# dobrosketchkun/dither_pie

Measured on AMD Instinct MI355X. Metric: Mpixel/s dither+quantize @4K 256-color (Bayer 8x8 + nearest-palette, uint8 RGB in/out), higher is better.
Workload: dtype u8; 1 GPU; C2: Bayer 8x8 + 256-colour nearest palette palr(256,7), 3840x2160 RGB, 24 distinct frames rnd(2160,3840,1234+i) per GPU resident in HBM, frames sharded per rank; frames_per_gpu=24, h=2160, w=3840, colors=256, matrix=8x8, parallelism=frames x1

## Files before the change

dither_pie_amd/csrc/host_sanitize.cpp:

```cpp
#include <cstdio>
#include <cstdlib>
#include <cstring>
#include <string>

#include "host_logic.h"
#include "ordered_plan.h"
#include "ordered_fine.h"

using namespace dp;

static std::vector<double> read_pts(const char *path, int K)
{
    std::vector<double> p((size_t)K * 3);
    FILE *f = fopen(path, "rb");
    if (!f || fread(p.data(), sizeof(double), p.size(), f) != p.size()) {
        fprintf(stderr, "cannot read %d points from %s\n", K, path);
        exit(2);
    }
    fclose(f);
    return p;
}

static uint32_t lcg(uint32_t &s)
{
// ... 623 lines not shown
    const int mw = 8;
    std::vector<uint32_t> coord4(K), tm, nm;
    for (int j = 0; j < K; ++j) coord4[j] = (uint32_t)pal[3 * j] | ((uint32_t)pal[3 * j + 1] << 8) | ((uint32_t)pal[3 * j + 2] << 16);
    fine_masks(pal, K, mw, tm, nm);
    FineTable ft, again;
    fine_pack(tm.data(), nm.data(), mw, K, coord4, fine_table_fits, ft);
    fine_pack(tm.data(), nm.data(), mw, K, coord4, fine_table_fits, again);
    const std::vector<uint32_t> im = ft.ok ? ft.lds_image() : std::vector<uint32_t>();
    int bad = ft.ok != again.ok || ft.off != again.off || ft.win_idx != again.win_idx || ft.wide_idx != again.wide_idx;
    if (ft.ok) bad += (int64_t)im.size() * 4 != fine_table_bytes(ft.n_win, ft.n_wide) || !fine_table_fits(ft.n_win, ft.n_wide);
    f = fopen(out_path, "wb");
    if (!f) return 2;
    const int32_t head[4] = {ft.ok ? 1 : 0, ft.n_win, ft.n_wide, (int32_t)im.size()};
    fwrite(head, sizeof(int32_t), 4, f);
    if (ft.ok) {
        fwrite(ft.off.data(), 2, ft.off.size(), f);
        fwrite(ft.win_idx.data(), 2, ft.win_idx.size(), f);
        fwrite(ft.wide_cell.data(), 2, ft.wide_cell.size(), f);
        fwrite(ft.wide_idx.data(), 2, ft.wide_idx.size(), f);
        fwrite(ft.quad.data(), 4, ft.quad.size(), f);
        fwrite(ft.pair.data(), 4, ft.pair.size(), f);
        fwrite(ft.wide.data(), 4, ft.wide.size(), f);
        fwrite(im.data(), 4, im.size(), f);
    }
    fclose(f);
    printf("finepack K=%d ok=%d windows=%d wide=%d bytes=%lld bad=%d\n", K, (int)ft.ok, ft.n_win, ft.n_wide,
           (long long)(ft.ok ? fine_table_bytes(ft.n_win, ft.n_wide) : 0), bad);
    return bad ? 1 : 0;
}

static int run_fineplan(const char *path, const int n_cases)
{
    FILE *f = fopen(path, "rb");
    if (!f) {
        fprintf(stderr, "cannot open %s\n", path);
        return 2;
    }
    for (int c = 0; c < n_cases; ++c) {
        OrderedFacts facts;
        OrderedSwitches sw;
        FineFacts ff;
        if (fread(&facts, sizeof(facts), 1, f) != 1 || fread(&sw, sizeof(sw), 1, f) != 1 || fread(&ff, sizeof(ff), 1, f) != 1 || facts.hw < 1 ||
            facts.w < 1 || facts.n_cus < 1) {
            fprintf(stderr, "bad record %d in %s\n", c, path);
            return 2;
        }
        const OrderedPlan p = plan_ordered(facts, sw);
        printf("fine %d %s %d\n", c, family_name(p.family), (int)fine_replaces(p, ff));
    }
    fclose(f);
    return 0;
}

static int run_voidcluster(const char *path, const int n_cases)
{
    FILE *f = fopen(path, "rb");
    if (!f) {
        fprintf(stderr, "cannot open %s\n", path);
        return 2;
    }
    for (int c = 0; c < n_cases; ++c) {
        int32_t head[4];
        if (fread(head, sizeof(int32_t), 4, f) != 4 || !vac_args_ok(head[0], head[1], head[3])) {
            fprintf(stderr, "bad record %d in %s\n", c, path);
            return 2;
        }
        const int n = head[0] * head[1];
        std::vector<uint16_t> ranks((size_t)n);
        std::vector<float> thr((size_t)n);
        int rounds = 0;
        vac_generate(head[0], head[1], (uint32_t)head[2], head[3], ranks.data(), &rounds);
        vac_thresholds(ranks.data(), n, thr.data());
        printf("ranks %d %d", c, rounds);
        for (int i = 0; i < n; ++i) printf(" %u", (unsigned)ranks[(size_t)i]);
        printf("\nthr %d", c);
        for (int i = 0; i < n; ++i) {
            uint32_t bits;
            std::memcpy(&bits, &thr[(size_t)i], sizeof(bits));
            printf(" %08x", bits);
        }
        printf("\n");
    }
    fclose(f);
    return 0;
}

static int run_metric(const char *path, const int n_cases)
{
    FILE *f = fopen(path, "rb");
    if (!f) {
        fprintf(stderr, "cannot open %s\n", path);
        return 2;
    }
    for (int c = 0; c < n_cases; ++c) {
        int32_t head[2];
        if (fread(head, sizeof(int32_t), 2, f) != 2 || head[0] < 1 || head[0] > 256 || head[1] < 0 || head[1] > (1 << 20)) {
            fprintf(stderr, "bad record %d in %s\n", c, path);
            return 2;
        }
        const int K = head[0], n = head[1];
        std::vector<float> pal((size_t)3 * K), thr((size_t)n);
        std::vector<uint8_t> rgb((size_t)3 * n);
        if (fread(pal.data(), sizeof(float), pal.size(), f) != pal.size() || fread(thr.data(), sizeof(float), thr.size(), f) != thr.size() ||
            fread(rgb.data(), 1, rgb.size(), f) != rgb.size() || !metric_palette_ok(pal.data(), K)) {
            fprintf(stderr, "bad record %d in %s\n", c, path);
            return 2;
// ... 32 lines not shown
            fprintf(stderr, "bad record %d in %s\n", c, path);
            return 2;
        }
        IdiffPlan p;
        const int rc = idiff_plan(dx.data(), dy.data(), wt.data(), head[0], head[1], head[2], p);
        printf("idiff %d %d %d %d", c, rc, p.n, p.skew);
        for (int k = 0; k < p.n; ++k) printf(" %u", (unsigned)p.q[k]);
        printf("\n");
    }
    fclose(f);
    return 0;
}

static int run_okfit(const char *path, const int n_cases)
{
    FILE *f = fopen(path, "rb");
    if (!f) {
        fprintf(stderr, "cannot open %s\n", path);
        return 2;
    }
    for (int c = 0; c < n_cases; ++c) {
        int32_t head[3];
        if (fread(head, sizeof(int32_t), 3, f) != 3 || head[0] < 0 || head[0] > (1 << 24)) {
            fprintf(stderr, "bad record %d in %s\n", c, path);
            return 2;
        }
        const size_t n = (size_t)head[0];
        std::vector<uint32_t> codes(n), counts(n);
        if (fread(codes.data(), sizeof(uint32_t), n, f) != n || fread(counts.data(), sizeof(uint32_t), n, f) != n) {
            fprintf(stderr, "bad record %d in %s\n", c, path);
            return 2;
        }
        const int K = head[1], rule = okfit_check(codes.data(), counts.data(), (int64_t)n, K, head[2]);
        printf("okfit %d %d", c, rule);
        if (!rule) {
            std::vector<uint8_t> pal((size_t)3 * K);
            std::vector<int32_t> centres((size_t)3 * K);
            int n_iter = 0;
            uint64_t distortion = 0;
            okfit_host(codes.data(), counts.data(), (int64_t)n, K, head[2], pal.data(), centres.data(), &n_iter, &distortion);
            printf(" %d %llu", n_iter, (unsigned long long)distortion);
            for (int i = 0; i < 3 * K; ++i) printf(" %u", (unsigned)pal[(size_t)i]);
            for (int i = 0; i < 3 * K; ++i) printf(" %d", centres[(size_t)i]);
        }
        printf("\n");
    }
    fclose(f);
    return 0;
}

int main(int argc, char **argv)
{
    if (argc < 4) {
        fprintf(stderr, "usage: %s kdtree|edtables|accel <pts.f64> <K> [bw]  |  mediancut <rgb.u8> <n> <depth>  |  indexmap <lists.bin> <n>  |  giflzw <cases.bin> <n>  |  pngdeflate|pngdyn|pngfile <cases.bin> <n>  |  orderedplan <cases.bin> <n>  |  voidcluster <cases.bin> <n>  |  metric <cases.bin> <n>  |  finepack <pal.u8> <K> <out.bin>  |  fineplan <cases.bin> <n>  |  idiffplan <cases.bin> <n>  |  okfit <cases.bin> <n>\n", argv[0]);
        return 2;
    }
    if (std::string(argv[1]) == "mediancut") return run_mediancut(argv[2], atol(argv[3]), argc > 4 ? atoi(argv[4]) : 4);
    if (std::string(argv[1]) == "indexmap") return run_indexmap(argv[2], atoi(argv[3]));
    if (std::string(argv[1]) == "giflzw") return run_giflzw(argv[2], atoi(argv[3]));
    if (std::string(argv[1]) == "pngdeflate") return run_pngdeflate(argv[2], atoi(argv[3]), false);
    if (std::string(argv[1]) == "pngdyn") return run_pngdeflate(argv[2], atoi(argv[3]), true);
    if (std::string(argv[1]) == "pngfile") return run_pngfile(argv[2], atoi(argv[3]));
    if (std::string(argv[1]) == "orderedplan") return run_orderedplan(argv[2], atoi(argv[3]));
    if (std::string(argv[1]) == "voidcluster") return run_voidcluster(argv[2], atoi(argv[3]));
    if (std::string(argv[1]) == "metric") return run_metric(argv[2], atoi(argv[3]));
    if (std::string(argv[1]) == "finepack") return argc > 4 ? run_finepack(argv[2], atoi(argv[3]), argv[4]) : 2;
    if (std::string(argv[1]) == "fineplan") return run_fineplan(argv[2], atoi(argv[3]));
    if (std::string(argv[1]) == "idiffplan") return run_idiffplan(argv[2], atoi(argv[3]));
    if (std::string(argv[1]) == "okfit") return run_okfit(argv[2], atoi(argv[3]));
    const int K = atoi(argv[3]);
    if (K < 1 || K > 1024) return 2;
    const std::vector<double> pts = read_pts(argv[2], K);
    const std::string cmd = argv[1];
    if (cmd == "kdtree") return run_kdtree(pts, K);
    if (cmd == "edtables") return run_edtables(pts, K);
    if (cmd == "accel") return run_accel(pts, K, argc > 4 ? atoi(argv[4]) : 8);
    return 2;
}
```

dither_pie_amd/csrc/ordered.hip:

```cpp
#include <type_traits>

#include "dp_internal.h"
#include "ordered_plan.h"
#include "ordered_fine.h"
#include "tree_query.hip.h"

namespace dp {

namespace {

constexpr int kListCap = 16384;
constexpr int kLdsTreeK = 256;
constexpr int kLdsTreeNodes = 512;
constexpr int kDrainAt = kListCap - kBlock * 64;

struct Geo {
    uint32_t n_px;
    uint32_t hw, w, h;
    double inv_hw, inv_w;
    int y0, x0;
    int ty0, tx0;
    int aligned;
    int neg2;
    uint32_t adv_y, adv_x;
// ... 1763 lines not shown
        drain_b(qb < 64u ? qb : 64u);
    }
}


__device__ __forceinline__ void cand6(const uint32_t x, const uint4 ca, const uint32_t c4, const uint32_t c5, const int neg2, int &m0,
                                      int &m1, int &m2)
{
    int n0, n1, n2, n3, n4, n5, p0, p1, p2, p3, p4, p5;
    asm volatile(
        "v_dot4_u32_u8 %[n0], %[c0], %[c0], 0\n\t"
        "v_dot4_u32_u8 %[p0], %[x], %[c0], 0\n\t"
        "v_dot4_u32_u8 %[n1], %[c1], %[c1], 0\n\t"
        "v_dot4_u32_u8 %[p1], %[x], %[c1], 0\n\t"
        "v_dot4_u32_u8 %[n2], %[c2], %[c2], 0\n\t"
        "v_dot4_u32_u8 %[p2], %[x], %[c2], 0\n\t"
        "v_dot4_u32_u8 %[n3], %[c3], %[c3], 0\n\t"
        "v_dot4_u32_u8 %[p3], %[x], %[c3], 0\n\t"
        "v_dot4_u32_u8 %[n4], %[c4], %[c4], 0\n\t"
        "v_dot4_u32_u8 %[p4], %[x], %[c4], 0\n\t"
        "v_dot4_u32_u8 %[n5], %[c5], %[c5], 0\n\t"
        "v_dot4_u32_u8 %[p5], %[x], %[c5], 0\n\t"
        "v_lshl_add_u32 %[n0], %[n0], 8, 0\n\t"
        "v_lshl_add_u32 %[n1], %[n1], 8, 4\n\t"
        "v_lshl_add_u32 %[n2], %[n2], 8, 8\n\t"
        "v_lshl_add_u32 %[n3], %[n3], 8, 12\n\t"
        "v_lshl_add_u32 %[n4], %[n4], 8, 16\n\t"
        "v_lshl_add_u32 %[n5], %[n5], 8, 20\n\t"
        "v_mad_i32_i24 %[n0], %[p0], %[ng], %[n0]\n\t"
        "v_mad_i32_i24 %[n1], %[p1], %[ng], %[n1]\n\t"
        "v_mad_i32_i24 %[n2], %[p2], %[ng], %[n2]\n\t"
        "v_mad_i32_i24 %[n3], %[p3], %[ng], %[n3]\n\t"
        "v_mad_i32_i24 %[n4], %[p4], %[ng], %[n4]\n\t"
        "v_mad_i32_i24 %[n5], %[p5], %[ng], %[n5]\n\t"
        "v_min3_i32 %[m0], %[n0], %[n1], %[n2]\n\t"
        "v_med3_i32 %[m1], %[n0], %[n1], %[n2]\n\t"
        "v_max3_i32 %[m2], %[n0], %[n1], %[n2]\n\t"
        "v_med3_i32 %[m2], %[m1], %[m2], %[n3]\n\t"
        "v_med3_i32 %[m1], %[m0], %[m1], %[n3]\n\t"
        "v_min_i32 %[m0], %[m0], %[n3]\n\t"
        "v_med3_i32 %[m2], %[m1], %[m2], %[n4]\n\t"
        "v_med3_i32 %[m1], %[m0], %[m1], %[n4]\n\t"
        "v_min_i32 %[m0], %[m0], %[n4]\n\t"
        "v_med3_i32 %[m2], %[m1], %[m2], %[n5]\n\t"
        "v_med3_i32 %[m1], %[m0], %[m1], %[n5]\n\t"
        "v_min_i32 %[m0], %[m0], %[n5]\n\t"
        : [n0] "=&v"(n0), [n1] "=&v"(n1), [n2] "=&v"(n2), [n3] "=&v"(n3), [n4] "=&v"(n4), [n5] "=&v"(n5), [p0] "=&v"(p0),
          [p1] "=&v"(p1), [p2] "=&v"(p2), [p3] "=&v"(p3), [p4] "=&v"(p4), [p5] "=&v"(p5), [m0] "=&v"(m0), [m1] "=&v"(m1),
          [m2] "=&v"(m2)
        : [x] "v"(x), [c0] "v"(ca.x), [c1] "v"(ca.y), [c2] "v"(ca.z), [c3] "v"(ca.w), [c4] "v"(c4), [c5] "v"(c5),
          [ng] "s"(neg2));
}

__device__ __forceinline__ uint32_t fine_cell_offset(const uint32_t x)
{
    return ((x >> 2) & 0x3eu) | ((x >> 5) & 0x7c0u) | ((x >> 8) & 0xf800u);
}

struct FineLds {
    uint32_t wide_at, pair_at, off_at, ids_at, thr_at;
};

template <int MODE>
__device__ __forceinline__ uint32_t fine_pixel_full(const uint32_t entry, const uint8_t *__restrict__ in, uint8_t *__restrict__ out,
                                                    unsigned long long *__restrict__ flags, const Geo &g, const PalDev &pal,
                                                    const ThrDev &thr, const uint32_t *s_words, const FineLds &at)
{
    const uint32_t mask = entry & 15u;
    const uint32_t p = (entry >> 4) * 4u + (uint32_t)__builtin_ctz(mask | 16u);
    const uint8_t *s_bytes = reinterpret_cast<const uint8_t *>(s_words);
    const uint8_t *b = in + (size_t)p * 3;
    const uint32_t x = (uint32_t)b[0] | ((uint32_t)b[1] << 8) | ((uint32_t)b[2] << 16);
    LeanThr th;
    pixel_threshold<MODE>(p, g, thr, s_words + at.thr_at / 4, 0.0f, 0.0f, 0.0f, th);
    const uint32_t cell2 = fine_cell_offset(x);
    uint32_t c = 0;
    bool done = false, slow = false;
    if (*reinterpret_cast<const uint16_t *>(s_bytes + at.off_at + cell2) == 0) {
        const uint16_t *ids = reinterpret_cast<const uint16_t *>(s_bytes + at.ids_at);
        const uint32_t cell = cell2 >> 1;
        uint32_t lo = 0;
#pragma unroll
        for (uint32_t step = kFineIds / 2; step != 0u; step >>= 1)
            if ((uint32_t)ids[lo + step] <= cell) lo += step;
        done = resolve_wide<MODE>(x, th, thr.sh, s_words + at.wide_at / 4 + lo * kWideList, kWideList, c);
    }
    if (!done) {
        bool hard;
        Leaf lf;
        leaf_find_global<8>(x, pal, lf);
        c = resolve_pixel<MODE, 8>(x, th, lf, g, pal, thr, nullptr, slow, hard);
    }
    uint8_t *o = out + (size_t)p * 3;
    o[0] = (uint8_t)c;
    o[1] = (uint8_t)(c >> 8);
    o[2] = (uint8_t)(c >> 16);
    if (slow) flag_slow_pixel(p, flags, g);
    const uint32_t rest = mask & (mask - 1u);
    return rest ? ((entry & ~15u) | rest) : 0u;
}

template <int MODE>
__global__ __launch_bounds__(kCellBlock, 4) void ordered_fine_kernel(const uint8_t *__restrict__ in, uint8_t *__restrict__ out,
                                                                    unsigned long long *__restrict__ flags, const Geo g,
                                                                    const PalDev pal, const ThrDev thr, const float sx, const float sy,
                                                                    const float sc, const uint32_t n_tiles)
{
    static_assert(MODE == 1, "integer thresholds in LDS only");
    (void)sx, (void)sy, (void)sc;
    __shared__ __align__(16) uint32_t smem[kLeanLdsWords];
    for (int i = threadIdx.x * 2; i < pal.fine_words; i += kCellBlock * 2)
        *reinterpret_cast<uint2 *>(&smem[i]) = *reinterpret_cast<const uint2 *>(&pal.fine_tab[i]);
    {
        const int n = thr.th_h * thr.tw_pad;
        for (int i = threadIdx.x; i < n; i += kCellBlock) smem[pal.fine_words + i] = thr.mpad[i];
    }
    __syncthreads();
    FineLds at;
    at.wide_at = (uint32_t)pal.fine_win * (kFineQuad * 4);
    at.pair_at = at.wide_at + (uint32_t)pal.fine_wide * (kWideList * 4);
    at.off_at = at.pair_at + (uint32_t)pal.fine_win * ((kFineWindow - kFineQuad) * 4);
    at.ids_at = at.off_at + kFineCells * 2;
    at.thr_at = at.ids_at + kFineIds * 2;
    const uint8_t *s_bytes = reinterpret_cast<const uint8_t *>(smem);
    const uint32_t lane = threadIdx.x & 63u;
    uint32_t *s_queue = smem + (kLeanLdsWords - kLeanQueueWords) + (threadIdx.x >> 6) * kLeanQueue;
    uint32_t qcount = 0;
    const uint3 *in3 = reinterpret_cast<const uint3 *>(in);
    uint3 *out3 = reinterpret_cast<uint3 *>(out);
    const uint32_t n_full = g.n_px >> 2;

    auto windows = [&](const uint32_t xq[4], uint32_t win[4]) {
#pragma unroll
        for (int q = 0; q < 4; ++q) win[q] = *reinterpret_cast<const uint16_t *>(s_bytes + at.off_at + fine_cell_offset(xq[q]));
    };
    auto drain = [&](const uint32_t n) {
        qcount -= n;
        __threadfence_block();
        uint32_t rest = 0u;
        if (lane < n) rest = fine_pixel_full<MODE>(s_queue[qcount + lane], in, out, flags, g, pal, thr, smem, at);
        queue_push(s_queue, qcount, rest != 0u, rest);
    };

    uint32_t tile = blockIdx.x;
    uint32_t fy = 0, fx = 0;
    uint3 wn = make_uint3(0u, 0u, 0u), wnn = make_uint3(0u, 0u, 0u);
    uint32_t xn[4], winn[4];
    if (tile < n_tiles) {
        const uint32_t gidx0 = tile * kCellBlock + threadIdx.x;
        if (gidx0 < n_full) wn = in3[gidx0];
        if (gidx0 * 4u < g.n_px) locate(g, gidx0 * 4u, fy, fx);
        const uint32_t gidx1 = gidx0 + gridDim.x * kCellBlock;
        if (tile + gridDim.x < n_tiles && gidx1 < n_full) wnn = in3[gidx1];
    }
    unpack4(wn, xn);
    windows(xn, winn);
    const bool use_cls = thr.has_cls != 0;
    uint32_t cls_word = 0, cls_shift = 0;
    auto tile_class = [&](const uint32_t ty, const uint32_t tx, const uint32_t gi) {
        cls_word = 0;
        cls_shift = 0;
        if (!use_cls) return;
        const uint32_t y0l = (uint32_t)__builtin_amdgcn_readfirstlane((int)ty), x0l = (uint32_t)__builtin_amdgcn_readfirstlane((int)tx);
        const uint32_t g0 = (uint32_t)__builtin_amdgcn_readfirstlane((int)gi);
        if (x0l + 256u > g.w || g0 + 64u > n_full) return;
        const uint32_t row = ((uint32_t)g.y0 + y0l) & (uint32_t)(thr.th_h - 1), col = ((uint32_t)g.x0 + x0l) & (uint32_t)(thr.th_w - 1);
        const uint32_t idx = row * (uint32_t)thr.th_w + col;
        cls_word = thr.cls_nib[idx >> 3];
        cls_shift = (idx & 7u) * 4u;
    };
    if (tile < n_tiles) tile_class(fy, fx, tile * kCellBlock + threadIdx.x);
    for (; tile < n_tiles; tile += gridDim.x) {
        const uint32_t gidx = tile * kCellBlock + threadIdx.x;
        uint32_t xq[4], win[4];
#pragma unroll
        for (int q = 0; q < 4; ++q) {
            xq[q] = xn[q];
            win[q] = winn[q];
        }
        const uint32_t cls = (cls_word >> cls_shift) & 15u;
        const uint32_t cy = fy, cx = fx;
        {
            unpack4(wnn, xn);
            windows(xn, winn);
            const uint32_t next = tile + gridDim.x, next2 = next + gridDim.x;
            const uint32_t gn = next * kCellBlock + threadIdx.x, gn2 = next2 * kCellBlock + threadIdx.x;
            wnn = make_uint3(0u, 0u, 0u);
            if (next2 < n_tiles && gn2 < n_full) wnn = in3[gn2];
            tile_advance(g, fy, fx);
            cls_word = 0;
            if (next < n_tiles) tile_class(fy, fx, gn);
        }
        clear_flags(flags, gidx, lane);
        bool rare[4] = {false, false, false, false};
        if (gidx < n_full) {
            uint4 ca[4];
#pragma unroll
            for (int q = 0; q < 4; ++q) ca[q] = *reinterpret_cast<const uint4 *>(s_bytes + (win[q] << 4));
            auto body = [&](auto cls_c) {
                constexpr uint32_t CLS = (uint32_t)decltype(cls_c)::value;
                uint32_t pb[4];
                uint2 cb[4];
#pragma unroll
                for (int q = 0; q < 4; ++q) {
                    if ((CLS >> q) & 1u) continue;
                    pb[q] = (win[q] << 3) + (at.pair_at - 16u);
                    cb[q] = *reinterpret_cast<const uint2 *>(s_bytes + pb[q] + 16u);
                }
                LeanThr th[4];
#pragma unroll
                for (int q = 0; q < 4; ++q) {
                    th[q].mt = 0;
                    th[q].t = 0.0f;
                }
                if (CLS != 15u) {
                    uint32_t row, col;
                    thr_pos(thr, (uint32_t)g.y0 + cy, (uint32_t)g.x0 + cx, row, col);
                    const uint32_t ta = row * (uint32_t)thr.tw_pad + col;
#pragma unroll
                    for (int q = 0; q < 4; ++q) {
                        if ((CLS >> q) & 1u) continue;
                        th[q].mt = *reinterpret_cast<const uint32_t *>(s_bytes + at.thr_at + (ta + q) * 4u);
                    }
                }
                const bool straddle = cx + 3u >= g.w;
                uint32_t col[4];
#pragma unroll
                for (int q = 0; q < 4; ++q) {
                    const uint32_t x = xq[q];
                    if ((CLS >> q) & 1u) {
                        int m0, m1;
                        cand4n(x, ca[q], g.neg2, m0, m1);
                        rare[q] = ((uint32_t)(m0 ^ m1) < (1u << kLocalBits)) | straddle;
                        col[q] = *reinterpret_cast<const uint32_t *>(s_bytes + ((win[q] << 4) | ((uint32_t)m0 & 0xfcu)));
                    } else {
                        int m0, m1, m2;
                        cand6(x, ca[q], cb[q].x, cb[q].y, g.neg2, m0, m1, m2);
                        const int a0 = m0 >> kLocalBits, a1 = m1 >> kLocalBits;
                        const bool tie = (a0 == a1) | ((uint32_t)(m1 ^ m2) < (1u << kLocalBits));
                        const int xx = (int)__builtin_amdgcn_udot4(x, x, 0u, false);
                        const uint32_t d0 = (uint32_t)(a0 + xx);
                        const uint32_t S = d0 + (uint32_t)a1 + (uint32_t)xx;
                        bool eq;
                        const bool nearest = lean_decide<MODE>(d0, S, th[q], thr.sh, eq);
                        rare[q] = tie | eq | straddle;
                        const uint32_t pos = (uint32_t)(nearest ? m0 : m1) & 0xfcu;
                        col[q] = *reinterpret_cast<const uint32_t *>(s_bytes + ((pos < 16u ? (win[q] << 4) : pb[q]) + pos));
                    }
                }
                out3[gidx] = pack4(col);
            };
            if (cls == 5u) body(std::integral_constant<int, 5>{});
            else if (cls == 10u) body(std::integral_constant<int, 10>{});
            else if (cls == 15u) body(std::integral_constant<int, 15>{});
            else body(std::integral_constant<int, 0>{});
        } else {
#pragma unroll
            for (int q = 0; q < 4; ++q) rare[q] = gidx * 4u + (uint32_t)q < g.n_px;
        }
        const uint32_t rmask = (rare[0] ? 1u : 0u) | (rare[1] ? 2u : 0u) | (rare[2] ? 4u : 0u) | (rare[3] ? 8u : 0u);
        const unsigned long long rb = __ballot(rmask != 0u);
        if (rb != 0ull) {
            if (rmask != 0u)
                s_queue[__builtin_amdgcn_mbcnt_hi((uint32_t)(rb >> 32), __builtin_amdgcn_mbcnt_lo((uint32_t)rb, qcount))] = (gidx << 4) | rmask;
            qcount += (uint32_t)__popcll(rb);
            while (qcount >= 64u) drain(64u);
        }
    }
    while (qcount != 0u) drain(qcount < 64u ? qcount : 64u);
}

constexpr int kFloatKeyGap = 128;

struct alignas(16) Cand3 {
    float x, y, z;
};

__device__ __forceinline__ int med3_i32(const int a, const int b, const int c)
{
    int r;
    asm("v_med3_i32 %0, %1, %2, %3" : "=v"(r) : "v"(a), "v"(b), "v"(c));
    return r;
}

template <int MODE>
__global__ __launch_bounds__(kCellBlock) void ordered_lean_float_kernel(const uint8_t *__restrict__ in,
                                                                        uint8_t *__restrict__ out,
                                                                        unsigned long long *__restrict__ flags,
                                                                        const Geo g, const PalDev pal, const ThrDev thr,
                                                                        const float sx, const float sy, const float sc,
// ... 579 lines not shown
__global__ void ign_field_kernel(float *__restrict__ out, const int h, const int w, const int y0, const int x0,
                                 const float sx, const float sy, const float sc)
{
    const int x = blockIdx.x * blockDim.x + threadIdx.x;
    const int y = blockIdx.y;
    if (x < w && y < h) out[(size_t)y * w + x] = ign_threshold(x0 + x, y0 + y, sx, sy, sc);
}

__global__ void resize_tables_kernel(int *__restrict__ xtab, int *__restrict__ ytab, const int w, const int ow,
                                     const int h, const int oh)
{
    const int which = threadIdx.x;
    if (which > 1) return;
    const int n_in = which ? h : w, n_out = which ? oh : ow;
    int *tab = which ? ytab : xtab;
    const double a = (double)n_in / (double)n_out;
    double xo = __dmul_rn(a, 0.5);
    for (int x = 0; x < n_out; ++x) {
        int v = (int)xo;
        tab[x] = v < n_in ? v : n_in - 1;
        xo = __dadd_rn(xo, a);
    }
}

__global__ void resize_nearest_kernel(const uint8_t *__restrict__ in, uint8_t *__restrict__ out, const int h,
                                      const int w, const int oh, const int ow, const int *__restrict__ xtab,
                                      const int *__restrict__ ytab)
{
    const int x = blockIdx.x * blockDim.x + threadIdx.x;
    const int y = blockIdx.y;
    const size_t f = blockIdx.z;
    if (x >= ow || y >= oh) return;
    const uint8_t *s = in + (f * h * w + (size_t)ytab[y] * w + xtab[x]) * 3;
    uint8_t *d = out + (f * oh * ow + (size_t)y * ow + x) * 3;
    d[0] = s[0];
    d[1] = s[1];
    d[2] = s[2];
}

int num_cus()
{
    static thread_local int cached_dev = -1, cached = 0;
    int dev = 0;
    if (hipGetDevice(&dev) != hipSuccess) return 256;
    if (dev != cached_dev) {
        int n = 0;
        if (hipDeviceGetAttribute(&n, hipDeviceAttributeMultiprocessorCount, dev) != hipSuccess || n <= 0) n = 256;
        cached = n;
        cached_dev = dev;
    }
    return cached;
}

static inline void trace_plan(const OrderedPlan &p, bool aligned, bool fine)
{
#ifdef DP_EXPERIMENTS
    if (std::getenv("DP_ORDERED_TRACE")) {
        constexpr const char *tables[] = {"plain8", "plain4", "warped"};
        fprintf(stderr, "dp_ordered_u8: pass 1 = %s (4-byte aligned frames: %d) mode=%d bw=%d adapt=%d warp=%d half=%d table=%s fix_big_queue=%d kernel=%s\n",
                family_name(p.family), aligned ? 1 : 0, p.mode, p.bw, p.adapt ? 1 : 0, p.warp ? 1 : 0, p.half ? 1 : 0, tables[p.table],
                p.fix_big_queue ? 1 : 0, fine ? "fine" : family_name(p.family));
    }
#else
    (void)p;
    (void)aligned;
    (void)fine;
#endif
}

using TileKernel = void (*)(const uint8_t *, uint8_t *, unsigned long long *, Geo, PalDev, ThrDev, float, float, float, uint32_t);
using BruteKernel = void (*)(const uint8_t *, uint8_t *, unsigned long long *, Geo, PalDev, ThrDev, float, float, float);
using FixKernel = void (*)(const uint8_t *, uint8_t *, const unsigned long long *, uint32_t, Geo, PalDev, ThrDev, float, float, float);

template <int M>
TileKernel tile_kernel_of(const OrderedPlan &p)
{
    switch (p.family) {
    case kFamCell:
        return ordered_cell_kernel<M>;
    case kFamFast:
        if (p.bw == 4) return ordered_fast_kernel<M, 4>;
        return ordered_fast_kernel<M, 8>;
    case kFamLean:
        if (p.warp && p.bw == 4) return ordered_lean_kernel<M, 4, false, true>;
        if (p.warp && p.adapt) return ordered_lean_kernel<M, 8, true, true>;
        if (p.warp) return ordered_lean_kernel<M, 8, false, true>;
        if (p.bw == 4 && p.half) return ordered_lean_kernel<M, 4, false, false, true>;
        if (p.bw == 4) return ordered_lean_kernel<M, 4, false, false>;
        if (p.adapt) return ordered_lean_kernel<M, 8, true, false>;
        return ordered_lean_kernel<M, 8, false, false>;
    case kFamCompact:
        if (p.warp && p.half) return ordered_compact_kernel<M, true, true>;
        if (p.warp) return ordered_compact_kernel<M, true, false>;
        if (p.half) return ordered_compact_kernel<M, false, true>;
        return ordered_compact_kernel<M, false, false>;
    case kFamLeanFloat:
        if constexpr (M != 1) return ordered_lean_float_kernel<M>;
        break;
    case kFamCompactFloat:
        if constexpr (M != 1) return ordered_compact_float_kernel<M>;
        break;
    case kFamBrute:
        break;
    }
    return nullptr;
}

TileKernel tile_kernel(const OrderedPlan &p)
{
    switch (p.mode) {
    case 0: return tile_kernel_of<0>(p);
    case 1: return tile_kernel_of<1>(p);
    case 2: return tile_kernel_of<2>(p);
    case 3: return tile_kernel_of<3>(p);
    }
    return nullptr;
}

BruteKernel brute_kernel(const OrderedPlan &p, const bool integer)
{
    switch (p.mode) {
    case 0: return integer ? ordered_int_kernel<0> : ordered_f64_kernel<0>;
    case 1: return integer ? ordered_int_kernel<1> : ordered_f64_kernel<1>;
    case 2: return integer ? ordered_int_kernel<2> : ordered_f64_kernel<2>;
    case 3: return integer ? ordered_int_kernel<3> : ordered_f64_kernel<3>;
    }
    return nullptr;
}

FixKernel fix_kernel(const OrderedPlan &p)
{
    const bool big = p.fix_big_queue;
    switch (p.fix_mode) {
    case 0: return big ? fixup_kernel<0, kQueueLarge> : fixup_kernel<0, kQueueSmall>;
    case 2: return big ? fixup_kernel<2, kQueueLarge> : fixup_kernel<2, kQueueSmall>;
    case 3: return big ? fixup_kernel<3, kQueueLarge> : fixup_kernel<3, kQueueSmall>;
    }
    return nullptr;
}

OrderedFacts facts_of(const PalDev &pal, const ThrDev &thr, const Geo &g, const int mode)
{
    return OrderedFacts{mode, pal.K, pal.is_integer, pal.n_inner,
                        g.n_px, g.hw, g.w,
                        g.y0, g.x0, g.aligned,
                        pal.cell_tab != nullptr, pal.tab_words, pal.tab_total,
                        pal.cell_tab4 != nullptr, pal.tab4_words,
                        pal.warp_tab != nullptr, pal.warp_words, pal.warp_total, pal.warp_bw, pal.warp_adapt,
                        pal.adapt, pal.cell_perm != nullptr, pal.cell_perm4 != nullptr, pal.n_wide, pal.n_wide4,
                        pal.comp_tab != nullptr, pal.comp_words, pal.comp_warp,
                        pal.ftab != nullptr, pal.ftab_words,
                        thr.m != nullptr, thr.mpad != nullptr, thr.fpad != nullptr, thr.th_h, thr.th_w, thr.tw_pad,
                        num_cus()};
}

}

int launch_ordered(const uint8_t *in, uint8_t *out, int64_t n_frames, int h, int w, int y0, int x0,
                   const PalDev &pal, int mode, const ThrDev *thr_in, float ign_scale, int ign_seed, void *ws,
                   size_t ws_bytes, hipStream_t s)
{
    (void)ws_bytes;
    const ThrDev thr = mode == DP_MODE_MATRIX ? *thr_in : no_thresholds();
    OrderedSwitches sw;
    sw.lean_no_half = exp_env("DP_LEAN_NO_HALF") != nullptr;
    sw.fast_all = exp_env("DP_FAST_ALL") != nullptr;
    sw.force_compact = exp_env("DP_FORCE_COMPACT") != nullptr;
    sw.no_compact_kernel = exp_env("DP_NO_COMPACT_KERNEL") != nullptr;
    sw.compact_no_half = exp_env("DP_COMPACT_NO_HALF") != nullptr;

    const float sx = (float)((double)ign_seed * 0.37), sy = (float)((double)ign_seed * 0.73);
    const int64_t hw = (int64_t)h * w;
    const int64_t max_frames = std::max<int64_t>(1, ((int64_t)1 << 30) / hw - 1);
    unsigned long long *fl = reinterpret_cast<unsigned long long *>(ws);
    const size_t dirty_off = ((size_t)((std::min(max_frames, n_frames) * hw + 255) / 256) * 32 + 768) & ~size_t(7);

    for (int64_t f0 = 0; f0 < n_frames; f0 += max_frames) {
        const int64_t nf = std::min(max_frames, n_frames - f0);
        const uint8_t *in_c = in + (size_t)f0 * hw * 3;
        uint8_t *out_c = out + (size_t)f0 * hw * 3;
        Geo g;
        g.n_px = (uint32_t)(nf * hw);
        g.hw = (uint32_t)hw;
        g.w = (uint32_t)w;
        g.h = (uint32_t)h;
        g.inv_hw = 1.0 / (double)hw;
        g.inv_w = 1.0 / (double)w;
        g.y0 = y0;
        g.x0 = x0;
        g.ty0 = y0 % thr.th_h;
        g.tx0 = x0 % thr.th_w;
        g.aligned = (((uintptr_t)in_c | (uintptr_t)out_c) & 3) == 0;
        g.neg2 = -(2 << kLocalBits);
        g.dirty = reinterpret_cast<uint32_t *>(reinterpret_cast<uint8_t *>(ws) + dirty_off);
        const OrderedPlan plan = plan_ordered(facts_of(pal, thr, g, mode), sw);
        g.adv_y = plan.adv_y;
        g.adv_x = plan.adv_x;
        const bool brute = plan.family == kFamBrute;
        const bool fine = fine_replaces(plan, FineFacts{pal.fine_tab != nullptr, pal.fine_win, pal.fine_wide, thr.th_h * thr.tw_pad * 4}) &&
                          !exp_env("DP_NO_FINE_KERNEL");
        const BruteKernel brute_k = brute ? brute_kernel(plan, pal.is_integer != 0) : nullptr;
        const TileKernel tile_k = brute ? nullptr : (fine ? ordered_fine_kernel<1> : tile_kernel(plan));
        const FixKernel fix_k = fix_kernel(plan);
        if ((brute ? brute_k == nullptr : tile_k == nullptr) || fix_k == nullptr) {
            set_error("dp_ordered_u8: no %s kernel for mode %d", family_name(plan.family), plan.mode);
            return DP_EUNSUPPORTED;
        }
        DP_HIP(hipMemsetAsync(g.dirty, 0, sizeof(uint32_t), s));
        ProfMark *pm = prof_begin(s);
        if (brute) {
            hipLaunchKernelGGL(brute_k, dim3(plan.grid), dim3(plan.block), 0, s, in_c, out_c, fl, g, pal, thr, sx, sy, ign_scale);
        } else {
            if (plan.family == kFamCell)
                DP_HIP(hipFuncSetAttribute(reinterpret_cast<const void *>(tile_k), hipFuncAttributeMaxDynamicSharedMemorySize, (int)plan.lds_bytes));
            PalDev pal1 = pal;
            if (plan.table == kTabWarped) {
                pal1.cell_tab = pal.warp_tab;
                pal1.tab_words = pal.warp_words;
                pal1.tab_total = pal.warp_total;
            } else if (plan.table == kTabPlain4) {
                pal1.cell_tab = pal.cell_tab4;
                pal1.tab_words = pal.tab4_words;
                pal1.tab_total = pal.tab4_words;
            }
            hipLaunchKernelGGL(tile_k, dim3(plan.grid), dim3(plan.block), plan.lds_bytes, s, in_c, out_c, fl, g, pal1, thr, sx, sy, ign_scale,
                               plan.n_tiles);
        }
        DP_HIP(hipGetLastError());
        trace_plan(plan, g.aligned, fine);
        prof_mid(pm, s);
        hipLaunchKernelGGL(fix_k, dim3(plan.fix_grid), dim3(kBlock), 0, s, in_c, out_c, fl, plan.n_words, g, pal, thr, sx, sy, ign_scale);
        prof_end(pm, s);
        DP_HIP(hipGetLastError());
    }
    return DP_OK;
}

int launch_ign_thresholds(float *out, int h, int w, int y0, int x0, float scale, int seed, hipStream_t s)
{
    const float sx = (float)((double)seed * 0.37), sy = (float)((double)seed * 0.73);
    if (h > 65535) {
        set_error("dp_ign_thresholds: h > 65535 not supported");
        return DP_EUNSUPPORTED;
    }
    hipLaunchKernelGGL(ign_field_kernel, dim3((w + 255) / 256, h), dim3(256), 0, s, out, h, w, y0, x0, sx, sy, scale);
    DP_HIP(hipGetLastError());
    return DP_OK;
}

int launch_resize_nearest(const uint8_t *in, uint8_t *out, int64_t n_frames, int h, int w, int oh, int ow,
                          hipStream_t s)
{
    if (oh > 65535 || n_frames > 65535) {
        set_error("dp_resize_nearest_u8: oh or n_frames > 65535 not supported");
        return DP_EUNSUPPORTED;
    }
    int *tabs = nullptr;
    DP_HIP(hipMallocAsync((void **)&tabs, sizeof(int) * ((size_t)ow + oh), s));
    hipLaunchKernelGGL(resize_tables_kernel, dim3(1), dim3(64), 0, s, tabs, tabs + ow, w, ow, h, oh);
    hipLaunchKernelGGL(resize_nearest_kernel, dim3((ow + 255) / 256, oh, (unsigned)n_frames), dim3(256), 0, s, in, out,
                       h, w, oh, ow, tabs, tabs + ow);
    hipError_t e = hipGetLastError();
    (void)hipFreeAsync(tabs, s);
    if (e != hipSuccess) return hip_fail(e, "resize launch");
    return DP_OK;
}

}
```

dither_pie_amd/csrc/ordered_fine.h:

```cpp
#pragma once
#include <cstdint>

#include "ordered_plan.h"

namespace dp {

constexpr int64_t fine_table_bytes(const int n_win, const int n_wide)
{
    return (int64_t)n_win * (kFineWindow * 4) + (int64_t)n_wide * kWideList * 4 + kFineCells * 2 + kFineIds * 2;
}
constexpr bool fine_table_fits(const int n_win, const int n_wide)
{
    return fine_table_bytes(n_win, n_wide) + 16 * 19 * 4 <= kLeanTabBytes;
}

struct FineFacts {
    int32_t present;
    int32_t n_win, n_wide;
    int32_t thr_bytes;
};

inline bool fine_replaces(const OrderedPlan &p, const FineFacts &f)
{
    return f.present != 0 && p.family == kFamLean && p.mode == 1 && p.bw == 8 && p.table == kTabPlain8 && !p.adapt && !p.warp && !p.half &&
           fine_table_bytes(f.n_win, f.n_wide) + (int64_t)f.thr_bytes <= kLeanTabBytes;
}

}
```

Before: 406,300 Mpixel/s.

## Precompute palette norm keys in LDS for the fine ordered-dither kernel

```diff
diff --git a/dither_pie_amd/csrc/host_sanitize.cpp b/dither_pie_amd/csrc/host_sanitize.cpp
--- a/dither_pie_amd/csrc/host_sanitize.cpp
+++ b/dither_pie_amd/csrc/host_sanitize.cpp
@@ -699,6 +699,26 @@
     return 0;
 }
 
+static int run_finekeys(const char *path, const int n_cases)
+{
+    FILE *f = fopen(path, "rb");
+    if (!f) {
+        fprintf(stderr, "cannot open %s\n", path);
+        return 2;
+    }
+    for (int c = 0; c < n_cases; ++c) {
+        FineFacts ff;
+        if (fread(&ff, sizeof(ff), 1, f) != 1 || ff.n_win < 0 || ff.thr_bytes < 0) {
+            fprintf(stderr, "bad record %d in %s\n", c, path);
+            fclose(f);
+            return 2;
+        }
+        printf("keys %d %d\n", c, fine_keys_level(ff));
+    }
+    fclose(f);
+    return 0;
+}
+
 static int run_voidcluster(const char *path, const int n_cases)
 {
     FILE *f = fopen(path, "rb");
@@ -837,7 +857,7 @@
 int main(int argc, char **argv)
 {
     if (argc < 4) {
-        fprintf(stderr, "usage: %s kdtree|edtables|accel <pts.f64> <K> [bw]  |  mediancut <rgb.u8> <n> <depth>  |  indexmap <lists.bin> <n>  |  giflzw <cases.bin> <n>  |  pngdeflate|pngdyn|pngfile <cases.bin> <n>  |  orderedplan <cases.bin> <n>  |  voidcluster <cases.bin> <n>  |  metric <cases.bin> <n>  |  finepack <pal.u8> <K> <out.bin>  |  fineplan <cases.bin> <n>  |  idiffplan <cases.bin> <n>  |  okfit <cases.bin> <n>\n", argv[0]);
+        fprintf(stderr, "usage: %s kdtree|edtables|accel <pts.f64> <K> [bw]  |  mediancut <rgb.u8> <n> <depth>  |  indexmap <lists.bin> <n>  |  giflzw <cases.bin> <n>  |  pngdeflate|pngdyn|pngfile <cases.bin> <n>  |  orderedplan <cases.bin> <n>  |  voidcluster <cases.bin> <n>  |  metric <cases.bin> <n>  |  finepack <pal.u8> <K> <out.bin>  |  fineplan <cases.bin> <n>  |  finekeys <cases.bin> <n>  |  idiffplan <cases.bin> <n>  |  okfit <cases.bin> <n>\n", argv[0]);
         return 2;
     }
     if (std::string(argv[1]) == "mediancut") return run_mediancut(argv[2], atol(argv[3]), argc > 4 ? atoi(argv[4]) : 4);
@@ -851,6 +871,7 @@
     if (std::string(argv[1]) == "metric") return run_metric(argv[2], atoi(argv[3]));
     if (std::string(argv[1]) == "finepack") return argc > 4 ? run_finepack(argv[2], atoi(argv[3]), argv[4]) : 2;
     if (std::string(argv[1]) == "fineplan") return run_fineplan(argv[2], atoi(argv[3]));
+    if (std::string(argv[1]) == "finekeys") return run_finekeys(argv[2], atoi(argv[3]));
     if (std::string(argv[1]) == "idiffplan") return run_idiffplan(argv[2], atoi(argv[3]));
     if (std::string(argv[1]) == "okfit") return run_okfit(argv[2], atoi(argv[3]));
     const int K = atoi(argv[3]);
diff --git a/dither_pie_amd/csrc/ordered.hip b/dither_pie_amd/csrc/ordered.hip
--- a/dither_pie_amd/csrc/ordered.hip
+++ b/dither_pie_amd/csrc/ordered.hip
@@ -1839,16 +1839,113 @@
           [ng] "s"(neg2));
 }
 
+__device__ __forceinline__ void cand4k(const uint32_t x, const uint4 ca, const uint4 na, const int neg2, int &m0, int &m1)
+{
+    int n0, n1, n2, n3, p0, p1, p2, p3;
+    asm volatile(
+        "v_dot4_u32_u8 %[p0], %[x], %[c0], 0\n\t"
+        "v_dot4_u32_u8 %[p1], %[x], %[c1], 0\n\t"
+        "v_dot4_u32_u8 %[p2], %[x], %[c2], 0\n\t"
+        "v_dot4_u32_u8 %[p3], %[x], %[c3], 0\n\t"
+        "v_mad_i32_i24 %[n0], %[p0], %[ng], %[k0]\n\t"
+        "v_mad_i32_i24 %[n1], %[p1], %[ng], %[k1]\n\t"
+        "v_mad_i32_i24 %[n2], %[p2], %[ng], %[k2]\n\t"
+        "v_mad_i32_i24 %[n3], %[p3], %[ng], %[k3]\n\t"
+        "v_min3_i32 %[m0], %[n0], %[n1], %[n2]\n\t"
+        "v_med3_i32 %[m1], %[n0], %[n1], %[n2]\n\t"
+        "v_med3_i32 %[m1], %[m0], %[m1], %[n3]\n\t"
+        "v_min_i32 %[m0], %[m0], %[n3]\n\t"
+        : [n0] "=&v"(n0), [n1] "=&v"(n1), [n2] "=&v"(n2), [n3] "=&v"(n3), [p0] "=&v"(p0), [p1] "=&v"(p1), [p2] "=&v"(p2),
+          [p3] "=&v"(p3), [m0] "=&v"(m0), [m1] "=&v"(m1)
+        : [x] "v"(x), [c0] "v"(ca.x), [c1] "v"(ca.y), [c2] "v"(ca.z), [c3] "v"(ca.w), [k0] "v"(na.x), [k1] "v"(na.y), [k2] "v"(na.z),
+          [k3] "v"(na.w), [ng] "s"(neg2));
+}
+
+template <int KEYS>
+__device__ __forceinline__ void cand6k(const uint32_t x, const uint4 ca, const uint4 na, const uint32_t c4, const uint32_t c5,
+                                       const uint32_t k4, const uint32_t k5, const int neg2, int &m0, int &m1, int &m2)
+{
+    int n0, n1, n2, n3, n4, n5, p0, p1, p2, p3, p4, p5;
+    if constexpr (KEYS == 1) {
+        (void)k4, (void)k5;
+        asm volatile(
+            "v_dot4_u32_u8 %[p0], %[x], %[c0], 0\n\t"
+            "v_dot4_u32_u8 %[p1], %[x], %[c1], 0\n\t"
+            "v_dot4_u32_u8 %[p2], %[x], %[c2], 0\n\t"
+            "v_dot4_u32_u8 %[p3], %[x], %[c3], 0\n\t"
+            "v_dot4_u32_u8 %[n4], %[c4], %[c4], 0\n\t"
+            "v_dot4_u32_u8 %[p4], %[x], %[c4], 0\n\t"
+            "v_dot4_u32_u8 %[n5], %[c5], %[c5], 0\n\t"
+            "v_dot4_u32_u8 %[p5], %[x], %[c5], 0\n\t"
+            "v_mad_i32_i24 %[n0], %[p0], %[ng], %[k0]\n\t"
+            "v_mad_i32_i24 %[n1], %[p1], %[ng], %[k1]\n\t"
+            "v_mad_i32_i24 %[n2], %[p2], %[ng], %[k2]\n\t"
+            "v_mad_i32_i24 %[n3], %[p3], %[ng], %[k3]\n\t"
+            "v_lshl_add_u32 %[n4], %[n4], 8, 16\n\t"
+            "v_lshl_add_u32 %[n5], %[n5], 8, 20\n\t"
+            "v_mad_i32_i24 %[n4], %[p4], %[ng], %[n4]\n\t"
+            "v_mad_i32_i24 %[n5], %[p5], %[ng], %[n5]\n\t"
+            "v_min3_i32 %[m0], %[n0], %[n1], %[n2]\n\t"
+            "v_med3_i32 %[m1], %[n0], %[n1], %[n2]\n\t"
+            "v_max3_i32 %[m2], %[n0], %[n1], %[n2]\n\t"
+            "v_med3_i32 %[m2], %[m1], %[m2], %[n3]\n\t"
+            "v_med3_i32 %[m1], %[m0], %[m1], %[n3]\n\t"
+            "v_min_i32 %[m0], %[m0], %[n3]\n\t"
+            "v_med3_i32 %[m2], %[m1], %[m2], %[n4]\n\t"
+            "v_med3_i32 %[m1], %[m0], %[m1], %[n4]\n\t"
+            "v_min_i32 %[m0], %[m0], %[n4]\n\t"
+            "v_med3_i32 %[m2], %[m1], %[m2], %[n5]\n\t"
+            "v_med3_i32 %[m1], %[m0], %[m1], %[n5]\n\t"
+            "v_min_i32 %[m0], %[m0], %[n5]\n\t"
+            : [n0] "=&v"(n0), [n1] "=&v"(n1), [n2] "=&v"(n2), [n3] "=&v"(n3), [n4] "=&v"(n4), [n5] "=&v"(n5), [p0] "=&v"(p0),
+              [p1] "=&v"(p1), [p2] "=&v"(p2), [p3] "=&v"(p3), [p4] "=&v"(p4), [p5] "=&v"(p5), [m0] "=&v"(m0), [m1] "=&v"(m1),
+              [m2] "=&v"(m2)
+            : [x] "v"(x), [c0] "v"(ca.x), [c1] "v"(ca.y), [c2] "v"(ca.z), [c3] "v"(ca.w), [c4] "v"(c4), [c5] "v"(c5), [k0] "v"(na.x),
+              [k1] "v"(na.y), [k2] "v"(na.z), [k3] "v"(na.w), [ng] "s"(neg2));
+    } else {
+        asm volatile(
+            "v_dot4_u32_u8 %[p0], %[x], %[c0], 0\n\t"
+            "v_dot4_u32_u8 %[p1], %[x], %[c1], 0\n\t"
+            "v_dot4_u32_u8 %[p2], %[x], %[c2], 0\n\t"
+            "v_dot4_u32_u8 %[p3], %[x], %[c3], 0\n\t"
+            "v_dot4_u32_u8 %[p4], %[x], %[c4], 0\n\t"
+            "v_dot4_u32_u8 %[p5], %[x], %[c5], 0\n\t"
+            "v_mad_i32_i24 %[n0], %[p0], %[ng], %[k0]\n\t"
+            "v_mad_i32_i24 %[n1], %[p1], %[ng], %[k1]\n\t"
+            "v_mad_i32_i24 %[n2], %[p2], %[ng], %[k2]\n\t"
+            "v_mad_i32_i24 %[n3], %[p3], %[ng], %[k3]\n\t"
+            "v_mad_i32_i24 %[n4], %[p4], %[ng], %[k4]\n\t"
+            "v_mad_i32_i24 %[n5], %[p5], %[ng], %[k5]\n\t"
+            "v_min3_i32 %[m0], %[n0], %[n1], %[n2]\n\t"
+            "v_med3_i32 %[m1], %[n0], %[n1], %[n2]\n\t"
+            "v_max3_i32 %[m2], %[n0], %[n1], %[n2]\n\t"
+            "v_med3_i32 %[m2], %[m1], %[m2], %[n3]\n\t"
+            "v_med3_i32 %[m1], %[m0], %[m1], %[n3]\n\t"
+            "v_min_i32 %[m0], %[m0], %[n3]\n\t"
+            "v_med3_i32 %[m2], %[m1], %[m2], %[n4]\n\t"
+            "v_med3_i32 %[m1], %[m0], %[m1], %[n4]\n\t"
+            "v_min_i32 %[m0], %[m0], %[n4]\n\t"
+            "v_med3_i32 %[m2], %[m1], %[m2], %[n5]\n\t"
+            "v_med3_i32 %[m1], %[m0], %[m1], %[n5]\n\t"
+            "v_min_i32 %[m0], %[m0], %[n5]\n\t"
+            : [n0] "=&v"(n0), [n1] "=&v"(n1), [n2] "=&v"(n2), [n3] "=&v"(n3), [n4] "=&v"(n4), [n5] "=&v"(n5), [p0] "=&v"(p0),
+              [p1] "=&v"(p1), [p2] "=&v"(p2), [p3] "=&v"(p3), [p4] "=&v"(p4), [p5] "=&v"(p5), [m0] "=&v"(m0), [m1] "=&v"(m1),
+              [m2] "=&v"(m2)
+            : [x] "v"(x), [c0] "v"(ca.x), [c1] "v"(ca.y), [c2] "v"(ca.z), [c3] "v"(ca.w), [c4] "v"(c4), [c5] "v"(c5), [k0] "v"(na.x),
+              [k1] "v"(na.y), [k2] "v"(na.z), [k3] "v"(na.w), [k4] "v"(k4), [k5] "v"(k5), [ng] "s"(neg2));
+    }
+}
+
 __device__ __forceinline__ uint32_t fine_cell_offset(const uint32_t x)
 {
     return ((x >> 2) & 0x3eu) | ((x >> 5) & 0x7c0u) | ((x >> 8) & 0xf800u);
 }
 
 struct FineLds {
-    uint32_t wide_at, pair_at, off_at, ids_at, thr_at;
+    uint32_t wide_at, norm_at, pair_at, off_at, ids_at, thr_at;
 };
 
-template <int MODE>
+template <int MODE, int KEYS>
 __device__ __forceinline__ uint32_t fine_pixel_full(const uint32_t entry, const uint8_t *__restrict__ in, uint8_t *__restrict__ out,
                                                     unsigned long long *__restrict__ flags, const Geo &g, const PalDev &pal,
                                                     const ThrDev &thr, const uint32_t *s_words, const FineLds &at)
@@ -1870,7 +1967,8 @@
 #pragma unroll
         for (uint32_t step = kFineIds / 2; step != 0u; step >>= 1)
             if ((uint32_t)ids[lo + step] <= cell) lo += step;
-        done = resolve_wide<MODE>(x, th, thr.sh, s_words + at.wide_at / 4 + lo * kWideList, kWideList, c);
+        if constexpr (KEYS == 0) done = resolve_wide<MODE>(x, th, thr.sh, s_words + at.wide_at / 4 + lo * kWideList, kWideList, c);
+        else done = resolve_wide<MODE>(x, th, thr.sh, pal.fine_tab + (uint32_t)pal.fine_win * kFineQuad + lo * kWideList, kWideList, c);
     }
     if (!done) {
         bool hard;
@@ -1887,7 +1985,7 @@
     return rest ? ((entry & ~15u) | rest) : 0u;
 }
 
-template <int MODE>
+template <int MODE, int KEYS>
 __global__ __launch_bounds__(kCellBlock, 4) void ordered_fine_kernel(const uint8_t *__restrict__ in, uint8_t *__restrict__ out,
                                                                     unsigned long long *__restrict__ flags, const Geo g,
                                                                     const PalDev pal, const ThrDev thr, const float sx, const float sy,
@@ -1895,20 +1993,51 @@
 {
     static_assert(MODE == 1, "integer thresholds in LDS only");
     (void)sx, (void)sy, (void)sc;
+    static_assert(KEYS >= 0 && KEYS <= 2, "key levels: ordered_fine.h");
     __shared__ __align__(16) uint32_t smem[kLeanLdsWords];
-    for (int i = threadIdx.x * 2; i < pal.fine_words; i += kCellBlock * 2)
-        *reinterpret_cast<uint2 *>(&smem[i]) = *reinterpret_cast<const uint2 *>(&pal.fine_tab[i]);
+    FineLds at;
+    if constexpr (KEYS == 0) {
+        for (int i = threadIdx.x * 2; i < pal.fine_words; i += kCellBlock * 2)
+            *reinterpret_cast<uint2 *>(&smem[i]) = *reinterpret_cast<const uint2 *>(&pal.fine_tab[i]);
+        at.wide_at = (uint32_t)pal.fine_win * (kFineQuad * 4);
+        at.norm_at = 0;
+        at.pair_at = at.wide_at + (uint32_t)pal.fine_wide * (kWideList * 4);
+        at.off_at = at.pair_at + (uint32_t)pal.fine_win * ((kFineWindow - kFineQuad) * 4);
+    } else {
+        constexpr int kPairRec = KEYS == 2 ? 4 : 2;
+        const int n_win = pal.fine_win;
+        const int pair_src = n_win * kFineQuad + pal.fine_wide * kWideList;
+        const int tail_src = pair_src + n_win * (kFineWindow - kFineQuad);
+        at.wide_at = 0;
+        at.norm_at = (uint32_t)n_win * (kFineQuad * 4);
+        at.pair_at = 2 * at.norm_at;
+        at.off_at = at.pair_at + (uint32_t)n_win * (kPairRec * 4);
+        for (int wi = threadIdx.x; wi < n_win; wi += kCellBlock) {
+            const uint4 c = *reinterpret_cast<const uint4 *>(&pal.fine_tab[wi * kFineQuad]);
+            *reinterpret_cast<uint4 *>(&smem[wi * 4]) = c;
+            *reinterpret_cast<uint4 *>(&smem[n_win * 4 + wi * 4]) =
+                make_uint4((__builtin_amdgcn_udot4(c.x, c.x, 0u, false) << kLocalBits), (__builtin_amdgcn_udot4(c.y, c.y, 0u, false) << kLocalBits) + 4u,
+                           (__builtin_amdgcn_udot4(c.z, c.z, 0u, false) << kLocalBits) + 8u, (__builtin_amdgcn_udot4(c.w, c.w, 0u, false) << kLocalBits) + 12u);
+            const uint2 b = *reinterpret_cast<const uint2 *>(&pal.fine_tab[pair_src + wi * 2]);
+            if constexpr (KEYS == 2)
+                *reinterpret_cast<uint4 *>(&smem[n_win * 8 + wi * 4]) =
+                    make_uint4(b.x, b.y, (__builtin_amdgcn_udot4(b.x, b.x, 0u, false) << kLocalBits) + 16u,
+                               (__builtin_amdgcn_udot4(b.y, b.y, 0u, false) << kLocalBits) + 20u);
+            else
+                *reinterpret_cast<uint2 *>(&smem[n_win * 8 + wi * 2]) = b;
+        }
+        uint32_t *s_tail = smem + at.off_at / 4;
+        for (int i = threadIdx.x * 2; i < (kFineCells + kFineIds) / 2; i += kCellBlock * 2)
+            *reinterpret_cast<uint2 *>(&s_tail[i]) = *reinterpret_cast<const uint2 *>(&pal.fine_tab[tail_src + i]);
+    }
+    at.ids_at = at.off_at + kFineCells * 2;
+    at.thr_at = at.ids_at + kFineIds * 2;
     {
         const int n = thr.th_h * thr.tw_pad;
-        for (int i = threadIdx.x; i < n; i += kCellBlock) smem[pal.fine_words + i] = thr.mpad[i];
+        const int thr_word = KEYS == 0 ? pal.fine_words : (int)(at.thr_at / 4);
+        for (int i = threadIdx.x; i < n; i += kCellBlock) smem[thr_word + i] = thr.mpad[i];
     }
     __syncthreads();
-    FineLds at;
-    at.wide_at = (uint32_t)pal.fine_win * (kFineQuad * 4);
-    at.pair_at = at.wide_at + (uint32_t)pal.fine_wide * (kWideList * 4);
-    at.off_at = at.pair_at + (uint32_t)pal.fine_win * ((kFineWindow - kFineQuad) * 4);
-    at.ids_at = at.off_at + kFineCells * 2;
-    at.thr_at = at.ids_at + kFineIds * 2;
     const uint8_t *s_bytes = reinterpret_cast<const uint8_t *>(smem);
     const uint32_t lane = threadIdx.x & 63u;
     uint32_t *s_queue = smem + (kLeanLdsWords - kLeanQueueWords) + (threadIdx.x >> 6) * kLeanQueue;
@@ -1925,7 +2054,7 @@
         qcount -= n;
         __threadfence_block();
         uint32_t rest = 0u;
-        if (lane < n) rest = fine_pixel_full<MODE>(s_queue[qcount + lane], in, out, flags, g, pal, thr, smem, at);
+        if (lane < n) rest = fine_pixel_full<MODE, KEYS>(s_queue[qcount + lane], in, out, flags, g, pal, thr, smem, at);
         queue_push(s_queue, qcount, rest != 0u, rest);
     };
 
@@ -1981,18 +2110,29 @@
         clear_flags(flags, gidx, lane);
         bool rare[4] = {false, false, false, false};
         if (gidx < n_full) {
-            uint4 ca[4];
-#pragma unroll
-            for (int q = 0; q < 4; ++q) ca[q] = *reinterpret_cast<const uint4 *>(s_bytes + (win[q] << 4));
+            constexpr int kPairShift = KEYS == 2 ? 4 : 3;
+            uint4 ca[4], na[4];
+#pragma unroll
+            for (int q = 0; q < 4; ++q) {
+                ca[q] = *reinterpret_cast<const uint4 *>(s_bytes + (win[q] << 4));
+                if constexpr (KEYS != 0) na[q] = *reinterpret_cast<const uint4 *>(s_bytes + ((win[q] << 4) + at.norm_at));
+            }
             auto body = [&](auto cls_c) {
                 constexpr uint32_t CLS = (uint32_t)decltype(cls_c)::value;
                 uint32_t pb[4];
-                uint2 cb[4];
+                uint2 cb[4], nb[4];
 #pragma unroll
                 for (int q = 0; q < 4; ++q) {
                     if ((CLS >> q) & 1u) continue;
-                    pb[q] = (win[q] << 3) + (at.pair_at - 16u);
-                    cb[q] = *reinterpret_cast<const uint2 *>(s_bytes + pb[q] + 16u);
+                    pb[q] = (win[q] << kPairShift) + (at.pair_at - 16u);
+                    if constexpr (KEYS == 2) {
+                        const uint4 v = *reinterpret_cast<const uint4 *>(s_bytes + pb[q] + 16u);
+                        cb[q] = make_uint2(v.x, v.y);
+                        nb[q] = make_uint2(v.z, v.w);
+                    } else {
+                        cb[q] = *reinterpret_cast<const uint2 *>(s_bytes + pb[q] + 16u);
+                        nb[q] = make_uint2(0u, 0u);
+                    }
                 }
                 LeanThr th[4];
 #pragma unroll
@@ -2017,12 +2157,14 @@
                     const uint32_t x = xq[q];
                     if ((CLS >> q) & 1u) {
                         int m0, m1;
-                        cand4n(x, ca[q], g.neg2, m0, m1);
+                        if constexpr (KEYS == 0) cand4n(x, ca[q], g.neg2, m0, m1);
+                        else cand4k(x, ca[q], na[q], g.neg2, m0, m1);
                         rare[q] = ((uint32_t)(m0 ^ m1) < (1u << kLocalBits)) | straddle;
                         col[q] = *reinterpret_cast<const uint32_t *>(s_bytes + ((win[q] << 4) | ((uint32_t)m0 & 0xfcu)));
                     } else {
                         int m0, m1, m2;
-                        cand6(x, ca[q], cb[q].x, cb[q].y, g.neg2, m0, m1, m2);
+                        if constexpr (KEYS == 0) cand6(x, ca[q], cb[q].x, cb[q].y, g.neg2, m0, m1, m2);
+                        else cand6k<KEYS>(x, ca[q], na[q], cb[q].x, cb[q].y, nb[q].x, nb[q].y, g.neg2, m0, m1, m2);
                         const int a0 = m0 >> kLocalBits, a1 = m1 >> kLocalBits;
                         const bool tie = (a0 == a1) | ((uint32_t)(m1 ^ m2) < (1u << kLocalBits));
                         const int xx = (int)__builtin_amdgcn_udot4(x, x, 0u, false);
@@ -2708,19 +2850,22 @@
     return cached;
 }
 
-static inline void trace_plan(const OrderedPlan &p, bool aligned, bool fine)
+static inline void trace_plan(const OrderedPlan &p, bool aligned, bool fine, int keys)
 {
 #ifdef DP_EXPERIMENTS
     if (std::getenv("DP_ORDERED_TRACE")) {
         constexpr const char *tables[] = {"plain8", "plain4", "warped"};
-        fprintf(stderr, "dp_ordered_u8: pass 1 = %s (4-byte aligned frames: %d) mode=%d bw=%d adapt=%d warp=%d half=%d table=%s fix_big_queue=%d kernel=%s\n",
+        char keys_s[16] = "";
+        if (fine) snprintf(keys_s, sizeof(keys_s), " keys=%d", keys);
+        fprintf(stderr, "dp_ordered_u8: pass 1 = %s (4-byte aligned frames: %d) mode=%d bw=%d adapt=%d warp=%d half=%d table=%s fix_big_queue=%d kernel=%s%s\n",
                 family_name(p.family), aligned ? 1 : 0, p.mode, p.bw, p.adapt ? 1 : 0, p.warp ? 1 : 0, p.half ? 1 : 0, tables[p.table],
-                p.fix_big_queue ? 1 : 0, fine ? "fine" : family_name(p.family));
+                p.fix_big_queue ? 1 : 0, fine ? "fine" : family_name(p.family), keys_s);
     }
 #else
     (void)p;
     (void)aligned;
     (void)fine;
+    (void)keys;
 #endif
 }
 
@@ -2773,6 +2918,18 @@
     return nullptr;
 }
 
+TileKernel fine_kernel(const int keys)
+{
+    switch (keys) {
+    case 0: return ordered_fine_kernel<1, 0>;
+    case 1: return ordered_fine_kernel<1, 1>;
+#ifdef DP_EXPERIMENTS
+    case 2: return ordered_fine_kernel<1, 2>;
+#endif
+    }
+    return nullptr;
+}
+
 BruteKernel brute_kernel(const OrderedPlan &p, const bool integer)
 {
     switch (p.mode) {
@@ -2853,10 +3010,13 @@
         g.adv_y = plan.adv_y;
         g.adv_x = plan.adv_x;
         const bool brute = plan.family == kFamBrute;
-        const bool fine = fine_replaces(plan, FineFacts{pal.fine_tab != nullptr, pal.fine_win, pal.fine_wide, thr.th_h * thr.tw_pad * 4}) &&
-                          !exp_env("DP_NO_FINE_KERNEL");
+        const FineFacts fine_facts{pal.fine_tab != nullptr, pal.fine_win, pal.fine_wide, thr.th_h * thr.tw_pad * 4};
+        const bool fine = fine_replaces(plan, fine_facts) && !exp_env("DP_NO_FINE_KERNEL");
+        int keys_cap = kFineKeysShipped;
+        if (const char *cap = exp_env("DP_FINE_KEYS_MAX")) keys_cap = std::min(2, std::max(0, std::atoi(cap)));
+        const int fine_keys = fine ? std::min(fine_keys_level(fine_facts), keys_cap) : 0;
         const BruteKernel brute_k = brute ? brute_kernel(plan, pal.is_integer != 0) : nullptr;
-        const TileKernel tile_k = brute ? nullptr : (fine ? ordered_fine_kernel<1> : tile_kernel(plan));
+        const TileKernel tile_k = brute ? nullptr : (fine ? fine_kernel(fine_keys) : tile_kernel(plan));
         const FixKernel fix_k = fix_kernel(plan);
         if ((brute ? brute_k == nullptr : tile_k == nullptr) || fix_k == nullptr) {
             set_error("dp_ordered_u8: no %s kernel for mode %d", family_name(plan.family), plan.mode);
@@ -2883,7 +3043,7 @@
                                plan.n_tiles);
         }
         DP_HIP(hipGetLastError());
-        trace_plan(plan, g.aligned, fine);
+        trace_plan(plan, g.aligned, fine, fine_keys);
         prof_mid(pm, s);
         hipLaunchKernelGGL(fix_k, dim3(plan.fix_grid), dim3(kBlock), 0, s, in_c, out_c, fl, plan.n_words, g, pal, thr, sx, sy, ign_scale);
         prof_end(pm, s);
diff --git a/dither_pie_amd/csrc/ordered_fine.h b/dither_pie_amd/csrc/ordered_fine.h
--- a/dither_pie_amd/csrc/ordered_fine.h
+++ b/dither_pie_amd/csrc/ordered_fine.h
@@ -26,4 +26,18 @@
            fine_table_bytes(f.n_win, f.n_wide) + (int64_t)f.thr_bytes <= kLeanTabBytes;
 }
 
+constexpr int64_t fine_keys_bytes(const int level, const int n_win)
+{
+    return (int64_t)n_win * (level == 2 ? 48 : 40) + kFineCells * 2 + kFineIds * 2;
 }
+inline int fine_keys_level(const FineFacts &f)
+{
+    if (f.present == 0) return 0;
+    for (int level = 2; level >= 1; --level)
+        if (fine_keys_bytes(level, f.n_win) + (int64_t)f.thr_bytes <= kLeanTabBytes) return level;
+    return 0;
+}
+
+constexpr int kFineKeysShipped = 1;
+
+}
```

New measurement: 416,800 Mpixel/s, median of 6. +2.6%, better.
